# qitianwu/DIFFormer

Hardware: NVIDIA B200
Metric: DIFFormer-layer node-updates/sec (full_attention_conv 'simple', N=132534 H=4 D=64 fp32 per GPU) (higher is better)
Workload: dtype f32

## Files before the change

difformer_b200/csrc/simple_lp_sm100.cu:

```cuda
#include <atomic>
#include <mutex>
#include <vector>

#include "simple_tc.cuh"

namespace dif {
namespace {

constexpr int kLpThreads = 12 * 32;
constexpr int kLpNodes = 32;
constexpr int kLpTile = kLpNodes * 128;
constexpr int kLpNS = 4;
constexpr int kLpQTile = 128 * 128;
constexpr int kLpNQ = 4;
constexpr int kLpOutBox = 32 * 128;
constexpr int kLpOutStage = 4 * 2 * kLpOutBox;

template <int H, bool W = false>
struct LpGeo {
    static constexpr int kStage = 3 * H * kLpTile;
    static constexpr int kSmem1 = kLpNS * kStage;
    static constexpr int kSmem2 = PLay<H, W>::kBBytes + kLpNQ * kLpQTile + kLpOutStage + H * kDim * 4;
    static constexpr int kSmem = (kSmem1 > kSmem2 ? kSmem1 : kSmem2) + 1024;
    static constexpr int kChunks = H * 8;
    static constexpr int kRowGroups = 256 / kChunks;
};

struct Bf16 {
    static constexpr int kFmt = 1;
    __device__ static __forceinline__ void unpack2(uint32_t w, float& a, float& b) { a = __uint_as_float(w << 16); b = __uint_as_float(w & 0xffff0000u); }
    __device__ static __forceinline__ uint32_t pack2(float a, float b) { return bf2_bits(a, b); }
};

__device__ __forceinline__ uint32_t make_idesc_fmt(int M, int N, int a_mn, int b_mn, int a_fmt, int b_fmt) {
    uint32_t d = 0;
    d |= 1u << 4;
    d |= (uint32_t)a_fmt << 7;
    d |= (uint32_t)b_fmt << 10;
    d |= (uint32_t)a_mn << 15;
    d |= (uint32_t)b_mn << 16;
    d |= (uint32_t)(N >> 3) << 17;
    d |= (uint32_t)(M >> 4) << 24;
    return d;
}

struct LpArgs {
    ReduceArgs1 r;
    unsigned long long* flags2;
    int store_hint, reverse, l2_hints, pf_tiles;
};

template <int H, class T, bool W = false>
__global__ void __launch_bounds__(kLpThreads, 1) simple_lp_kernel(const __grid_constant__ LpArgs la, const __grid_constant__ CUtensorMap mq,
                                                                 const __grid_constant__ CUtensorMap mk, const __grid_constant__ CUtensorMap mv,
                                                                 const __grid_constant__ CUtensorMap mo) {
    using G = Geo<H>;
    using L = LpGeo<H, W>;
    using P = PLay<H, W>;
    const ReduceArgs1& a = la.r;
    extern __shared__ uint8_t smem_raw[];
    uint8_t* base = (uint8_t*)(((uintptr_t)smem_raw + 1023) & ~(uintptr_t)1023);
    uint8_t* Bop = base;
    uint8_t* qring = base + P::kBBytes;
    uint8_t* ostage = qring + kLpNQ * kLpQTile;
    float* us = reinterpret_cast<float*>(ostage + kLpOutStage);
    __shared__ uint64_t full[kLpNS], empty[kLpNS], done;
    __shared__ uint64_t qfull[kLpNQ], qempty[kLpNQ], tfull[kNAcc], tempty[kNAcc], bbar;
    __shared__ uint32_t tmem_slot;
    __shared__ float part[16];
    __shared__ __align__(16) float red[H == 1 ? 64 * 65 : 4096];
    const int tid = threadIdx.x, warp = tid >> 5, lane = tid & 31;
    const int64_t r0 = (int64_t)blockIdx.x * a.rows_per_cta;
    const int64_t r1 = min(a.N, r0 + (int64_t)a.rows_per_cta);
    const int iters = r1 > r0 ? (int)((r1 - r0 + kLpNodes - 1) / kLpNodes) : 0;
    const int my_tiles = r1 > r0 ? (int)((r1 - r0 + kTile2 - 1) / kTile2) : 0;
    const int nsc = my_tiles * H;
    auto row0_of = [&](int sc) -> int64_t { const int t = sc / H; return r0 + (int64_t)(la.reverse ? my_tiles - 1 - t : t) * kTile2; };
    uint64_t* dbg = a.dbg;
    DIF_STAMP(dbg, 0);

    if (tid == 0) {
        for (int s = 0; s < kLpNS; ++s) { mbar_init(&full[s], 1); mbar_init(&empty[s], 9); }
// ... 165 lines not shown
                __syncwarp();
                if (lane == 0) mbar_arrive(&empty[s]);
            }
        }
        ssk = warp_sum(ssk);
        ssq = warp_sum(ssq);
        if (lane == 0) { part[warp - 4] = ssk; part[8 + warp - 4] = ssq; }
#pragma unroll
        for (int i = 0; i < 8; ++i) { red[ts * 16 + i] = z[i]; red[ts * 16 + 8 + i] = u[i]; }
        __threadfence_block();
        if (warp >= 8) {
            bar_arrive_named(1, 256);
        } else {
            const int te = tid - 128, ew = warp - 4;
            mbar_wait(&done, 0);
            tc_fence_after();
            bar_sync_named(1, 256);
            if (dbg != nullptr && te == 0) dbg[blockIdx.x * kDbgSlots + 4] = gtime();
            float* rec = a.ws + (int64_t)blockIdx.x * a.ws_len;
            for (int col = te; col < H * kDim; col += 128) {
                const int ccid = col >> 3, e = col & 7;
                float zs = 0.f, usum = 0.f;
                for (int g = 0; g < L::kRowGroups; ++g) { zs += red[(g * L::kChunks + ccid) * 16 + e]; usum += red[(g * L::kChunks + ccid) * 16 + 8 + e]; }
                rec[P::offZ + col] = zs;
                rec[P::offU + col] = usum;
            }
            if (te == 0) {
                float sk = 0.f, sq = 0.f;
                for (int w = 0; w < 8; ++w) { sk += part[w]; sq += part[8 + w]; }
                rec[P::offSq] = sq;
                rec[P::offSq + 1] = sk;
            }
            if (H == 1) bar_sync_named(2, 128);
            const int64_t pf_rows = min((int64_t)min(la.pf_tiles, my_tiles) * kTile2, r1 - r0);
            fused_tail<H, W>(a, la.flags2, rec, te, ew, lane, tmem, iters > 0, red, reinterpret_cast<const __nv_bfloat16*>(a.q) + r0 * (H * kDim),
                          (uint32_t)(max((int64_t)0, pf_rows) * H * kDim * 2));
            if (te == 0) {
                mbar_expect_tx(&bbar, (uint32_t)P::kBBytes);
                for (int i = 0; i < P::kBTiles * 2; ++i)
                    tma_load_1d(smem_u32(Bop) + i * kBOp, a.prepared + (size_t)i * kBOp, (uint32_t)kBOp, &bbar);
            }
            for (int i = te; i < H * kDim; i += 128) us[i] = __ldcg(a.partials + P::offU + i);
            const float cscale = 1.f / (sqrtf(__ldcg(a.partials + P::offSq)) * sqrtf(__ldcg(a.partials + P::offSq + 1)));
            bar_sync_named(2, 128);
            const uint32_t obox = smem_u32(ostage) + ew * 2 * kLpOutBox;
            const uint64_t pol = policy_evict_first();
            float inv_den = 0.f;
            for (int sc = 0; sc < nsc; ++sc) {
                const int64_t trow = row0_of(sc);
                const int h = sc % H, slot = sc % kNAcc;
                mbar_wait(&tfull[slot], (sc / kNAcc) & 1);
                tc_fence_after();
                const uint32_t taddr = tmem + ((uint32_t)(ew * 32) << 16) + slot * kAccCols;
                if (!W || h == 0) {
                    uint32_t qz_bits = tmem_ld1(taddr + kDim);
                    tmem_ld_wait1(qz_bits);
                    inv_den = 1.f / (fmaf(__uint_as_float(qz_bits), cscale, a.n_total));
                }
                const uint32_t ob = obox + (sc & 1) * kLpOutBox;
                if (lane == 0) tma_wait_read1();
                __syncwarp();
#pragma unroll
                for (int c0 = 0; c0 < kDim; c0 += 32) {
                    uint32_t r[32];
                    tmem_ld32(taddr + c0, r);
                    tmem_ld_wait32(r);
                    if (c0 == 32) {
                        tc_fence_before();
                        __syncwarp();
// ... 79 lines not shown
int simple_forward_lp(const void* q, const void* k, const void* v, int dtype, int64_t N, int H, int Hv, int M, int D, double n_total,
                      float* partials, void* out, void* ws, int64_t ws_bytes, cudaStream_t st,
                      void* const* peer_bufs, int rank, int world, unsigned long long seq) {
    const bool wide = simple_wide_supported(N, H, Hv, M, D);
    DIF_REQUIRE(wide || simple_tc_supported(N, H, Hv, M, D), DIF_EUNSUPPORTED, "tcgen05 path: unsupported shape");
    DIF_REQUIRE(dtype == DIF_DTYPE_BF16, DIF_EUNSUPPORTED, "simple_forward(16-bit): bf16 only (dtype %d): up-cast fp16 and use the fp32 kernel", dtype);
    DIF_REQUIRE((((uintptr_t)q | (uintptr_t)k | (uintptr_t)v | (uintptr_t)out) & 15) == 0, DIF_EARG, "simple_forward(16-bit): q/k/v/out must be 16-byte aligned");
    DIF_REQUIRE(((uintptr_t)ws & 127) == 0, DIF_EARG, "simple_forward: workspace must be 128-byte aligned");
    DIF_REQUIRE(N < (1ll << 31), DIF_EUNSUPPORTED, "tcgen05 path: N must fit a 32-bit TMA coordinate");
    int grid;
    const int rpc = tc_rows_per_cta(N, H, &grid);
    const int64_t ws_len = wide ? PLay<2, true>::kWsLen : tc_ws_len(H);
    const int64_t poff = fused_ws_prepared_off(grid, ws_len);
    DIF_REQUIRE(ws_bytes >= poff + (wide ? (int64_t)PLay<2, true>::kBBytes : (int64_t)H * 2 * kBOp), DIF_EARG, "simple_forward: workspace too small");
    DIF_REQUIRE((((ws_len + kSlices - 1) / kSlices + 3) & ~(int64_t)3) <= 128, DIF_EUNSUPPORTED, "simple_forward: slice wider than the tail warps");
    static std::atomic<unsigned long long> epoch_src{0x5851F42D4C957F2Dull ^ (unsigned long long)(uintptr_t)&epoch_src};
    LpArgs la{};
    ReduceArgs1& a = la.r;
    a.N = N; a.rows_per_cta = rpc;
    a.ws = (float*)ws; a.ws_len = ws_len; a.flags = (unsigned long long*)((char*)ws + fused_ws_flags_off(grid, ws_len));
    la.flags2 = a.flags + (int64_t)(grid + 1) * kFlagStride;
    a.epoch = epoch_src.fetch_add(0x632BE59BD9B4E019ull) | 1ull;
    a.partials = partials; a.prepared = (uint8_t*)ws + poff;
    a.n_total = (float)n_total;
    a.sh.world = 1;
    if (peer_bufs != nullptr && world > 1) {
        DIF_REQUIRE(world <= kCommMaxRanks && rank >= 0 && rank < world && seq > 0, DIF_EARG, "simple_forward(sharded): bad rank/world/seq");
        for (int r = 0; r < world; ++r) { DIF_REQUIRE(peer_bufs[r], DIF_EARG, "simple_forward(sharded): null peer buffer"); a.sh.bufs[r] = peer_bufs[r]; }
        a.sh.rank = rank; a.sh.world = world; a.sh.seq = seq;
        a.sh.lenpad = comm_lenpad(SimpleLayout{H, Hv, M, D}.len());
        a.sh.timeout_ns = comm_timeout_ns();
    }
    static const int hints = env_int("DIF_TC_P1_HINTS", 1), sth = env_int("DIF_TC_P2_STORE_HINT", 1), rev = env_int("DIF_TC_FUSED_REVERSE", 1);
    static const int pft = env_int("DIF_TC_FUSED_PF_TILES", 0);
    la.l2_hints = hints; la.store_hint = sth; la.reverse = rev; la.pf_tiles = pft;
    a.q = reinterpret_cast<const float*>(q);
    a.dbg = dbg_buffer();
    const int fp16 = 0;
    CUtensorMap maps[4];
    int rc;
    if ((rc = make_map16(&maps[0], q, N, (int64_t)H * M, fp16))) return rc;
    if ((rc = make_map16(&maps[1], k, N, (int64_t)H * M, fp16))) return rc;
    if ((rc = make_map16(&maps[2], v, N, (int64_t)H * D, fp16))) return rc;
    if ((rc = make_map16(&maps[3], out, N, (int64_t)H * D, fp16))) return rc;
#define DIF_LP(T) (H == 4 ? launch_lp<4, T>(la, maps, grid, st) : H == 2 ? launch_lp<2, T>(la, maps, grid, st) : launch_lp<1, T>(la, maps, grid, st))
    rc = wide ? launch_lp<2, Bf16, true>(la, maps, grid, st) : DIF_LP(Bf16);
#undef DIF_LP
    if (rc) return rc;
    dbg_report("simple_lp", a.dbg, grid);
    return DIF_OK;
}

}
```

difformer_b200/csrc/simple_sm100.cu:

```cuda
#include <stdlib.h>

#include <atomic>
#include <mutex>
#include <vector>

#include "simple_tc.cuh"

namespace dif {

int simple_finalize_fwd(const float* ws, int nchunks, int H, int Hv, int M, int D, float* partials, cudaStream_t st);

namespace {

template <int H, bool BWD>
__global__ void __launch_bounds__(kThreadsT, 1) reduce_tma_kernel(const __grid_constant__ ReduceArgs1 a) {
    using G = Geo<H>;
    extern __shared__ uint8_t smem_raw[];
    uint8_t* stg = (uint8_t*)(((uintptr_t)smem_raw + 1023) & ~(uintptr_t)1023);
    uint8_t* ops = stg + G::kNSG * G::kStg;
    __shared__ uint64_t sfull[G::kNSG], sempty[G::kNSG], ofull[G::kNO], oempty[G::kNO], done, tail_bar;
    __shared__ uint32_t tmem_slot;
    __shared__ float part[16];
    __shared__ __align__(16) float szc[BWD ? H * kDim : 4], su[BWD ? H * kDim : 4];
    const int tid = threadIdx.x, warp = tid >> 5, lane = tid & 31;
// ... 1076 lines not shown
            for (int ks = 0; ks < 4; ++ks) {
                const uint64_t ahi = make_desc(sb + ks * 32, kKmajLBO, kKmajSBO), alo = make_desc(sb + kQOp + ks * 32, kKmajLBO, kKmajSBO);
                const uint64_t bhi = make_desc(bb + ks * 32, kKmajLBO, kKmajSBO), blo = make_desc(bb + kBOpB + ks * 32, kKmajLBO, kKmajSBO);
                umma(d, ahi, bhi, idesc, ks > 0 ? 1u : 0u);
                umma(d, alo, bhi, idesc, 1u);
                umma(d, ahi, blo, idesc, 1u);
            }
            umma_commit(&empty[s]);
            umma_commit(&tfull[slot]);
        }
    }
    __syncwarp();
    tc_fence_before();
    __syncthreads();
    if (warp == 12) tmem_dealloc(tmem, 512);
}


template <int H, bool W = false>
__global__ void __launch_bounds__(kThreadsTC, 1) simple_fused_kernel(const __grid_constant__ FusedArgs fa, const __grid_constant__ CUtensorMap out_map) {
    using G = Geo<H>;
    using P = PLay<H, W>;
    const ReduceArgs1& a = fa.r;
    extern __shared__ uint8_t smem_raw[];
    uint8_t* base = (uint8_t*)(((uintptr_t)smem_raw + 1023) & ~(uintptr_t)1023);
    uint8_t* stg = base;
    uint8_t* ops = stg + G::kNSG * G::kStg;
    uint8_t* Bop = base;
    uint8_t* stages = base + P::kBBytes;
    uint8_t* ostage = stages + kNS2 * kStage2;
    float* us = reinterpret_cast<float*>(ostage + kOutStage);
    __shared__ uint64_t sfull[G::kNSG], sempty[G::kNSG], ofull[G::kNO], oempty[G::kNO], done;
    __shared__ uint64_t full[kNS2], empty[kNS2], tfull[kNAcc], tempty[kNAcc], bbar;
    __shared__ uint32_t tmem_slot;
    __shared__ float part[16];
    __shared__ __align__(16) float red[H == 1 ? 64 * 65 : 2048];
    const int tid = threadIdx.x, warp = tid >> 5, lane = tid & 31;
    const int64_t r0 = (int64_t)blockIdx.x * a.rows_per_cta;
    const int64_t r1 = min(a.N, r0 + (int64_t)a.rows_per_cta);
    const int iters = r1 > r0 ? (int)((r1 - r0 + G::kNodes - 1) / G::kNodes) : 0;
    const int my_tiles = r1 > r0 ? (int)((r1 - r0 + kTile2 - 1) / kTile2) : 0;
    const int nsc = my_tiles * H;
    auto row0_of = [&](int sc) -> int64_t { const int t = sc / H; return r0 + (int64_t)(fa.reverse ? my_tiles - 1 - t : t) * kTile2; };
    uint64_t* dbg = a.dbg;
    DIF_STAMP(dbg, 0);

    if (tid == 0) {
        for (int s = 0; s < G::kNSG; ++s) { mbar_init(&sfull[s], 1); mbar_init(&sempty[s], 8); }
        for (int s = 0; s < G::kNO; ++s) { mbar_init(&ofull[s], 8); mbar_init(&oempty[s], 1); }
        mbar_init(&done, 1);
        for (int s = 0; s < kNS2; ++s) { mbar_init(&full[s], 8); mbar_init(&empty[s], 1); }
        for (int s = 0; s < kNAcc; ++s) { mbar_init(&tfull[s], 1); mbar_init(&tempty[s], 4); }
        mbar_init(&bbar, 1);
        asm volatile("fence.mbarrier_init.release.cluster;" ::: "memory");
    }
    if (warp == 12) tmem_alloc(&tmem_slot, 512);
    tc_fence_before();
    __syncthreads();
    tc_fence_after();
    const uint32_t tmem = tmem_slot;
    pdl_wait();
    DIF_STAMP(dbg, 1);

    if (warp < 8) {
        float zacc[4] = {0.f, 0.f, 0.f, 0.f}, uacc[4] = {0.f, 0.f, 0.f, 0.f};
        float ssk = 0.f, ssq = 0.f;
        {
            const uint32_t stg_base = smem_u32(stg), ops_base = smem_u32(ops);
            for (int it = 0; it < iters; ++it) {
                const int s = it % G::kNSG, o = it % G::kNO;
                const int nrows = (int)min((int64_t)G::kNodes, r1 - (r0 + (int64_t)it * G::kNodes));
                mbar_wait(&sfull[s], (it / G::kNSG) & 1);
                float4 x[G::kChunksPerThread][3];
#pragma unroll
                for (int i = 0; i < G::kChunksPerThread; ++i) {
                    const int u = tid + 256 * i, node = u / G::kChunksPerRow;
#pragma unroll
                    for (int t = 0; t < 3; ++t) {
                        x[i][t] = make_float4(0.f, 0.f, 0.f, 0.f);
                        if (node < nrows) x[i][t] = lds128(stg_base + s * G::kStg + t * G::kStgT + u * 16);
                    }
                }
                if (it >= G::kNO) mbar_wait(&oempty[o], ((it / G::kNO) - 1) & 1);
                const uint32_t ob = ops_base + o * G::kOpStage;
#pragma unroll
                for (int i = 0; i < G::kChunksPerThread; ++i) {
                    const int u = tid + 256 * i, node = u / G::kChunksPerRow, cc = u % G::kChunksPerRow;
                    const int head = cc >> 4, m = (cc & 15) * 4;
                    const int blk = (H == 1) ? (node >> 4) : head;
                    const int kn = (H == 1) ? (node & 15) : node;
                    const uint32_t off = (uint32_t)(blk * G::kBlockTile + (kn >> 3) * 1024 + (kn & 7) * 128 +
                                                    ((((m >> 3) ^ kn) & 7) << 4) + ((m >> 2) & 1) * 8);
                    uint32_t hi[2], lo[2];
                    split4(x[i][0], hi, lo);
                    sts64(ob + 0 * G::kOp + off, hi[0], hi[1]);
                    sts64(ob + 1 * G::kOp + off, lo[0], lo[1]);
                    split4(x[i][1], hi, lo);
                    sts64(ob + 2 * G::kOp + off, hi[0], hi[1]);
                    sts64(ob + 3 * G::kOp + off, lo[0], lo[1]);
                    const float4 kk = x[i][0], vv = x[i][1], qq = x[i][2];
                    zacc[0] += kk.x; zacc[1] += kk.y; zacc[2] += kk.z; zacc[3] += kk.w;
                    uacc[0] += vv.x; uacc[1] += vv.y; uacc[2] += vv.z; uacc[3] += vv.w;
                    ssk = fmaf(kk.x, kk.x, ssk); ssk = fmaf(kk.y, kk.y, ssk); ssk = fmaf(kk.z, kk.z, ssk); ssk = fmaf(kk.w, kk.w, ssk);
                    ssq = fmaf(qq.x, qq.x, ssq); ssq = fmaf(qq.y, qq.y, ssq); ssq = fmaf(qq.z, qq.z, ssq); ssq = fmaf(qq.w, qq.w, ssq);
                }
                fence_proxy_async();
                __syncwarp();
                if (lane == 0) { mbar_arrive(&ofull[o]); mbar_arrive(&sempty[s]); }
            }
        }
        ssk = warp_sum(ssk);
        ssq = warp_sum(ssq);
        if (lane == 0) { part[warp] = ssk; part[8 + warp] = ssq; }
#pragma unroll
        for (int i = 0; i < 4; ++i) { red[tid * 4 + i] = zacc[i]; red[1024 + tid * 4 + i] = uacc[i]; }
        __threadfence_block();
        bar_arrive_named(1, 384);
        float buf[2][4][8];
        auto issue = [&](int sc, int j, float (&dst)[8]) {
            if (sc >= nsc) return;
            const int t = tid + 256 * j;
            const int64_t row = row0_of(sc) + (t >> 3);
            if (row < r1) {
                ldg256_stream(a.q + row * G::kRowF + (sc % H) * kDim + (t & 7) * 8, dst);
            } else {
#pragma unroll
                for (int i = 0; i < 8; ++i) dst[i] = 0.f;
            }
        };
#pragma unroll
        for (int j = 0; j < 4; ++j) issue(0, j, buf[0][j]);
#pragma unroll
        for (int j = 0; j < 4; ++j) issue(1, j, buf[1][j]);
        mbar_wait(&done, 0);
        DIF_STAMP(dbg, 3);
        const uint32_t stage_base = smem_u32(stages);
        for (int sc = 0; sc < nsc; ++sc) {
            const int s = sc % kNS2;
            if (sc >= kNS2) mbar_wait(&empty[s], ((sc / kNS2) - 1) & 1);
            const uint32_t sb = stage_base + s * kStage2;
#pragma unroll
            for (int j = 0; j < 4; ++j) {
                const int t = tid + 256 * j;
                uint4 hi, lo;
                split8(buf[0][j], hi, lo);
                const uint32_t off = sw128(t >> 3, t & 7);
                sts128(sb + off, hi);
                sts128(sb + kQOp + off, lo);
            }
            fence_proxy_async();
            __syncwarp();
            if (lane == 0) mbar_arrive(&full[s]);
#pragma unroll
            for (int j = 0; j < 4; ++j) {
#pragma unroll
                for (int i = 0; i < 8; ++i) buf[0][j][i] = buf[1][j][i];
                issue(sc + 2, j, buf[1][j]);
            }
        }
    } else if (warp < 12) {
        const int te = tid - 256, ew = warp - 8;
        if (warp == 8 && lane == 0) {
            const uint32_t stg_base = smem_u32(stg);
            const uint64_t pol_first = policy_evict_first_(), pol_last = policy_evict_last();
            for (int it = 0; it < iters; ++it) {
                const int s = it % G::kNSG;
                if (it >= G::kNSG) mbar_wait(&sempty[s], ((it / G::kNSG) - 1) & 1);
                const int64_t row = r0 + (int64_t)it * G::kNodes;
                const uint32_t bytes = (uint32_t)(min((int64_t)G::kNodes, r1 - row) * G::kRowB);
                mbar_expect_tx(&sfull[s], 3 * bytes);
                if (a.l2_hints) {
                    tma_load_1d_hint(stg_base + s * G::kStg + 0 * G::kStgT, a.k + row * G::kRowF, bytes, &sfull[s], pol_first);
                    tma_load_1d_hint(stg_base + s * G::kStg + 1 * G::kStgT, a.v + row * G::kRowF, bytes, &sfull[s], pol_first);
                    tma_load_1d_hint(stg_base + s * G::kStg + 2 * G::kStgT, a.q + row * G::kRowF, bytes, &sfull[s], pol_last);
                } else {
                    tma_load_1d(stg_base + s * G::kStg + 0 * G::kStgT, a.k + row * G::kRowF, bytes, &sfull[s]);
                    tma_load_1d(stg_base + s * G::kStg + 1 * G::kStgT, a.v + row * G::kRowF, bytes, &sfull[s]);
                    tma_load_1d(stg_base + s * G::kStg + 2 * G::kStgT, a.q + row * G::kRowF, bytes, &sfull[s]);
                }
            }
        }
        __syncwarp();
        mbar_wait(&done, 0);
        tc_fence_after();
        bar_sync_named(1, 384);
        if (dbg != nullptr && te == 0) dbg[blockIdx.x * kDbgSlots + 4] = gtime();
        float* rec = a.ws + (int64_t)blockIdx.x * a.ws_len;
        for (int col = te; col < G::kRowF; col += 128) {
            float z = 0.f, u = 0.f;
            for (int t = col >> 2; t < 256; t += G::kChunksPerRow) { z += red[t * 4 + (col & 3)]; u += red[1024 + t * 4 + (col & 3)]; }
            rec[P::offZ + col] = z;
            rec[P::offU + col] = u;
        }
        if (te == 0) {
            float sk = 0.f, sq = 0.f;
            for (int w = 0; w < 8; ++w) { sk += part[w]; sq += part[8 + w]; }
            rec[P::offSq] = sq;
            rec[P::offSq + 1] = sk;
        }
        if (H == 1) bar_sync_named(2, 128);
        const int64_t pf_rows = min((int64_t)min(fa.pf_tiles, my_tiles) * kTile2, r1 - r0);
        fused_tail<H, W>(a, fa.flags2, rec, te, ew, lane, tmem, iters > 0, red, a.q + r0 * G::kRowF, (uint32_t)(max((int64_t)0, pf_rows) * G::kRowB));
        if (te == 0) {
            mbar_expect_tx(&bbar, (uint32_t)P::kBBytes);
            for (int i = 0; i < P::kBTiles * 2; ++i)
                tma_load_1d(smem_u32(Bop) + i * kBOp, a.prepared + (size_t)i * kBOp, (uint32_t)kBOp, &bbar);
        }
        for (int i = te; i < H * kDim; i += 128) us[i] = __ldcg(a.partials + P::offU + i);
        const float cscale = 1.f / (sqrtf(__ldcg(a.partials + P::offSq)) * sqrtf(__ldcg(a.partials + P::offSq + 1)));
        bar_sync_named(2, 128);
        const uint32_t obox = smem_u32(ostage) + ew * 2 * kOutBox;
        const uint64_t pol = policy_evict_first();
        float inv_den = 0.f;
        for (int sc = 0; sc < nsc; ++sc) {
            const int64_t trow = row0_of(sc);
            const int h = sc % H, slot = sc % kNAcc;
            mbar_wait(&tfull[slot], (sc / kNAcc) & 1);
            tc_fence_after();
            const uint32_t taddr = tmem + ((uint32_t)(ew * 32) << 16) + slot * kAccCols;
            if (!W || h == 0) {
                uint32_t qz_bits = tmem_ld1(taddr + kDim);
                tmem_ld_wait1(qz_bits);
                inv_den = 1.f / (fmaf(__uint_as_float(qz_bits), cscale, a.n_total));
            }
            if (lane == 0) tma_wait_read0();
            __syncwarp();
#pragma unroll
            for (int c0 = 0; c0 < kDim; c0 += 32) {
                uint32_t r[32];
                tmem_ld32(taddr + c0, r);
                tmem_ld_wait32(r);
                if (c0 == 32) {
                    tc_fence_before();
                    __syncwarp();
                    if (lane == 0) mbar_arrive(&tempty[slot]);
                }
#pragma unroll
                for (int j = 0; j < 32; j += 4) {
                    const float4 u4 = *reinterpret_cast<const float4*>(us + h * kDim + c0 + j);
                    float4 o;
                    o.x = fmaf(__uint_as_float(r[j]), cscale, u4.x) * inv_den;
                    o.y = fmaf(__uint_as_float(r[j + 1]), cscale, u4.y) * inv_den;
                    o.z = fmaf(__uint_as_float(r[j + 2]), cscale, u4.z) * inv_den;
// ... 271 lines not shown
    } else if (shared_a) {
        rc = H == 4 ? launch_apply<4, true>(a, map, grid, st) : launch_apply<2, true>(a, map, grid, st);
    } else {
        rc = H == 4 ? launch_apply<4>(a, map, grid, st) : H == 2 ? launch_apply<2>(a, map, grid, st) : launch_apply<1>(a, map, grid, st);
    }
    if (rc) return rc;
    dbg_report("apply_tc", a.dbg, grid);
    return DIF_OK;
}


bool simple_wide_supported(int64_t N, int H, int Hv, int M, int D) { return N >= 1 && H == 1 && Hv == 1 && M == 128 && D == 128; }

int64_t simple_fused_workspace_bytes(int64_t N, int H, int Hv, int M, int D) {
    const bool wide = simple_wide_supported(N, H, Hv, M, D);
    if (!wide && !simple_tc_supported(N, H, Hv, M, D)) return 0;
    int grid;
    tc_rows_per_cta(N, H, &grid);
    const int64_t ws_len = wide ? PLay<2, true>::kWsLen : tc_ws_len(H);
    return fused_ws_prepared_off(grid, ws_len) + (wide ? (int64_t)PLay<2, true>::kBBytes : (int64_t)H * 2 * kBOp) + 128;
}

template <int H, bool W = false>
static int launch_fused(const FusedArgs& a, const CUtensorMap& map, int grid, cudaStream_t st) {
    static bool attr_set = false;
    if (!attr_set) {
        DIF_CUDA_OK(cudaFuncSetAttribute(simple_fused_kernel<H, W>, cudaFuncAttributeMaxDynamicSharedMemorySize, smem_fused_bytes<H, W>()));
        attr_set = true;
    }
    void* args[] = {(void*)&a, (void*)&map};
    return launch_persistent((const void*)simple_fused_kernel<H, W>, grid, kThreadsTC, (size_t)smem_fused_bytes<H, W>(), st, args);
}

int simple_forward_tc(const float* q, const float* k, const float* v, int64_t N, int H, int Hv, int M, int D, double n_total,
                      float* partials, float* out, void* ws, int64_t ws_bytes, cudaStream_t st,
                      void* const* peer_bufs, int rank, int world, unsigned long long seq) {
    const bool wide = simple_wide_supported(N, H, Hv, M, D);
    DIF_REQUIRE(wide || simple_tc_supported(N, H, Hv, M, D), DIF_EUNSUPPORTED, "tcgen05 path: unsupported shape");
    DIF_REQUIRE((((uintptr_t)q | (uintptr_t)k | (uintptr_t)v) & 31) == 0 && ((uintptr_t)out & 15) == 0, DIF_EARG, "simple_forward: q/k/v must be 32-byte, out 16-byte aligned");
    DIF_REQUIRE(((uintptr_t)ws & 127) == 0, DIF_EARG, "simple_forward: workspace must be 128-byte aligned");
    DIF_REQUIRE(N < (1ll << 31), DIF_EUNSUPPORTED, "tcgen05 path: N must fit a 32-bit TMA coordinate");
    int grid;
    const int rpc = tc_rows_per_cta(N, H, &grid);
    const int64_t ws_len = wide ? PLay<2, true>::kWsLen : tc_ws_len(H);
    const int64_t poff = fused_ws_prepared_off(grid, ws_len);
    DIF_REQUIRE(ws_bytes >= poff + (wide ? (int64_t)PLay<2, true>::kBBytes : (int64_t)H * 2 * kBOp), DIF_EARG, "simple_forward: workspace too small");
    DIF_REQUIRE((((ws_len + kSlices - 1) / kSlices + 3) & ~(int64_t)3) <= 128, DIF_EUNSUPPORTED, "simple_forward: slice wider than the tail warps");
    static std::atomic<unsigned long long> epoch_src{0xA24BAED4963EE407ull ^ (unsigned long long)(uintptr_t)&epoch_src};
    FusedArgs fa{};
    ReduceArgs1& a = fa.r;
    a.q = q; a.k = k; a.v = v; a.N = N; a.rows_per_cta = rpc;
    a.ws = (float*)ws; a.ws_len = ws_len; a.flags = (unsigned long long*)((char*)ws + fused_ws_flags_off(grid, ws_len));
    fa.flags2 = a.flags + (int64_t)(grid + 1) * kFlagStride;
    a.epoch = epoch_src.fetch_add(0x632BE59BD9B4E019ull) | 1ull;
    a.partials = partials; a.prepared = (uint8_t*)ws + poff;
    a.vbar = nullptr;
    static const int hints = env_int("DIF_TC_P1_HINTS", 1), sth = env_int("DIF_TC_P2_STORE_HINT", 1), rev = env_int("DIF_TC_FUSED_REVERSE", 1);
    static const int pft = env_int("DIF_TC_FUSED_PF_TILES", 0);
    a.l2_hints = hints;
    fa.pf_tiles = pft;
    a.n_total = (float)n_total;
    a.sh.world = 1;
    if (peer_bufs != nullptr && world > 1) {
        DIF_REQUIRE(world <= kCommMaxRanks && rank >= 0 && rank < world && seq > 0, DIF_EARG, "simple_forward(sharded): bad rank/world/seq");
        for (int r = 0; r < world; ++r) { DIF_REQUIRE(peer_bufs[r], DIF_EARG, "simple_forward(sharded): null peer buffer"); a.sh.bufs[r] = peer_bufs[r]; }
        a.sh.rank = rank; a.sh.world = world; a.sh.seq = seq;
        a.sh.lenpad = comm_lenpad(SimpleLayout{H, Hv, M, D}.len());
        a.sh.timeout_ns = comm_timeout_ns();
    }
    a.dbg = dbg_buffer();
    fa.out = out; fa.store_hint = sth; fa.reverse = rev;
    CUtensorMap map;
    int rc = make_out_map(&map, out, N, (int64_t)H * D);
    if (rc) return rc;
    rc = wide ? launch_fused<2, true>(fa, map, grid, st)
       : H == 4 ? launch_fused<4>(fa, map, grid, st) : H == 2 ? launch_fused<2>(fa, map, grid, st) : launch_fused<1>(fa, map, grid, st);
    if (rc) return rc;
    dbg_report("simple_fused", a.dbg, grid);
    return DIF_OK;
}

int64_t simple_tc_rowscal_floats(int64_t N, int H) { return N * H * 2; }

int simple_bwd_reduce_tc(const float* q, const float* g, const float* out, const float* partials, double n_total,
                         int64_t N, int H, float* bwd_partials, float* rowscal, void* ws, int64_t ws_bytes, cudaStream_t st) {
    DIF_REQUIRE(simple_tc_supported(N, H, H, kDim, kDim), DIF_EUNSUPPORTED, "tcgen05 path: unsupported shape");
    DIF_REQUIRE((((uintptr_t)q | (uintptr_t)g | (uintptr_t)out) & 15) == 0 && ((uintptr_t)rowscal & 7) == 0, DIF_EARG, "tcgen05 bwd: misaligned pointer");
    int grid;
    const int rpc = tc_rows_per_cta(N, H, &grid);
    const int64_t ws_len = tc_ws_len(H);
    DIF_REQUIRE(ws_bytes >= (int64_t)grid * ws_len * 4 + (int64_t)(grid + 1) * 8, DIF_EARG, "simple_bwd_reduce(tcgen05): workspace too small");
    static std::atomic<unsigned long long> epoch_src{0xD1B54A32D192ED03ull ^ (unsigned long long)(uintptr_t)&epoch_src};
    ReduceArgs1 a{};
// ... 59 lines not shown
```

difformer_b200/csrc/simple_tc.cuh:

```cuda
#pragma once
#include <stdlib.h>

#include "common.cuh"
#include "tc_ptx.cuh"

namespace dif {
namespace {

template <int H>
struct Geo {
    static_assert(H == 1 || H == 2 || H == 4, "tcgen05 path: H in {1, 2, 4}");
    static constexpr int kRowF = H * kDim;
    static constexpr int kRowB = kRowF * 4;
    static constexpr int kBlocks = H < 2 ? 2 : H;
    static constexpr int kPairs = kBlocks / 2;
    static constexpr int kNodes = 16 * kBlocks / H;
    static constexpr int kBlockTile = 16 * 128;
    static constexpr int kOp = kBlocks * kBlockTile;
    static constexpr int kOpStage = 4 * kOp;
    static constexpr int kStgT = kNodes * kRowB;
    static constexpr int kStg = 3 * kStgT;
    static constexpr int kNSG = 3, kNO = 2;
    static constexpr int kSmem1 = kNSG * kStg + kNO * kOpStage + 1024;
    static constexpr int kChunksPerRow = kRowB / 16;
// ... 26 lines not shown
    float* ws;
    int64_t ws_len;
    unsigned long long* flags;
    unsigned long long epoch;
    float* partials;
    uint8_t* prepared;
    int l2_hints;
    ShardArgs sh;
    uint64_t* dbg;
    const float* fwd_partials;
    float n_total;
    float* rowscal;
    float* vbar;
    int gram;
};


constexpr int kTile2 = 128;
constexpr int kQOp = kTile2 * 128;
constexpr int kStage2 = 2 * kQOp;
constexpr int kNS2 = 3;
constexpr int kBN = 80;
constexpr int kNAcc = 4, kAccCols = 128;
constexpr int kOutBox = 32 * 128;
constexpr int kOutStage = 4 * 2 * kOutBox;
template <int H>
constexpr int smem2_bytes() { return Geo<H>::kBBytes + kNS2 * kStage2 + kOutStage + H * kDim * 4 + 1024; }


struct FusedArgs {
    ReduceArgs1 r;
    float* out;
    int store_hint, reverse;
    int pf_tiles;
    unsigned long long* flags2;
};
template <int H, bool W = false>
constexpr int smem_fused_bytes() {
    constexpr int p2 = PLay<H, W>::kBBytes + kNS2 * kStage2 + kOutStage + H * kDim * 4 + 1024;
    return Geo<H>::kSmem1 > p2 ? Geo<H>::kSmem1 : p2;
}

__device__ __forceinline__ void bar_sync_named(int id, int nthreads) { asm volatile("bar.sync %0, %1;" :: "r"(id), "r"(nthreads) : "memory"); }
__device__ __forceinline__ void bar_arrive_named(int id, int nthreads) { asm volatile("bar.arrive %0, %1;" :: "r"(id), "r"(nthreads) : "memory"); }


int tc_grid(int64_t units) {
    const int sms = sm_count();
    return (int)(units < sms ? (units < 1 ? 1 : units) : sms);
}

int tc_rows_per_cta(int64_t N, int H, int* grid) {
    (void)H;
    int g = tc_grid((N + kTile2 - 1) / kTile2);
    int64_t rpc = (N + g - 1) / g;
    rpc = (rpc + kTile2 - 1) / kTile2 * kTile2;
    g = (int)((N + rpc - 1) / rpc);
    *grid = g;
    return (int)rpc;
}

uint64_t* dbg_buffer() {
    static uint64_t* buf = nullptr;
    static int on = -1;
    if (on < 0) { const char* e = getenv("DIF_TC_DEBUG_TIMES"); on = (e && atoi(e)) ? 1 : 0; }
    if (!on) return nullptr;
    if (!buf) cudaMalloc(&buf, 256 * kDbgSlots * sizeof(uint64_t));
    cudaMemset(buf, 0, 256 * kDbgSlots * sizeof(uint64_t));
// ... 49 lines not shown
        return DIF_OK;
    }
    if (mode == 3) {
        cudaLaunchConfig_t cfg{};
        cfg.gridDim = dim3(grid); cfg.blockDim = dim3(threads); cfg.dynamicSmemBytes = smem; cfg.stream = st;
        cudaLaunchAttribute attr[2];
        attr[0].id = cudaLaunchAttributeCooperative;
        attr[0].val.cooperative = 1;
        attr[1].id = cudaLaunchAttributeProgrammaticStreamSerialization;
        attr[1].val.programmaticStreamSerializationAllowed = 1;
        cfg.attrs = attr; cfg.numAttrs = 2;
        DIF_CUDA_OK(cudaLaunchKernelExC(&cfg, kernel, args));
        return DIF_OK;
    }
    int nb = 0;
    DIF_CUDA_OK(cudaOccupancyMaxActiveBlocksPerMultiprocessor(&nb, kernel, threads, smem));
    DIF_REQUIRE(nb >= 1 && grid <= sm_count(), DIF_ECUDA, "persistent kernel cannot be co-resident (grid %d, %d CTA/SM)", grid, nb);
    cudaLaunchConfig_t cfg{};
    cfg.gridDim = dim3(grid); cfg.blockDim = dim3(threads); cfg.dynamicSmemBytes = smem; cfg.stream = st;
    cudaLaunchAttribute attr[1];
    attr[0].id = cudaLaunchAttributeProgrammaticStreamSerialization;
    attr[0].val.programmaticStreamSerializationAllowed = 1;
    cfg.attrs = attr; cfg.numAttrs = mode == 2 ? 1 : 0;
    DIF_CUDA_OK(cudaLaunchKernelExC(&cfg, kernel, args));
    return DIF_OK;
}
__device__ __forceinline__ void pdl_wait() { asm volatile("griddepcontrol.wait;" ::: "memory"); }
__device__ __forceinline__ void pdl_launch_dependents() { asm volatile("griddepcontrol.launch_dependents;" ::: "memory"); }

int64_t tc_ws_len(int H) { return (SimpleLayout{H, H, kDim, kDim}.len() + 7) & ~(int64_t)7; }

constexpr int kFlagStride = 16;
int64_t fused_ws_flags_off(int grid, int64_t ws_len) { return ((int64_t)grid * ws_len * 4 + 127) & ~(int64_t)127; }
int64_t fused_ws_prepared_off(int grid, int64_t ws_len) { return fused_ws_flags_off(grid, ws_len) + (int64_t)(2 * grid + 1) * kFlagStride * 8; }


__device__ __forceinline__ void poll_flags(const unsigned long long* flags, int grid, int l, unsigned long long epoch) {
    constexpr int kMax = 8;
    bool ok;
    do {
        unsigned long long f[kMax];
#pragma unroll
        for (int i = 0; i < kMax; ++i) {
            const int r = l + 32 * i;
            f[i] = epoch;
            if (r < grid) asm volatile("ld.relaxed.gpu.global.u64 %0, [%1];" : "=l"(f[i]) : "l"(flags + (int64_t)r * kFlagStride) : "memory");
        }
        ok = true;
#pragma unroll
        for (int i = 0; i < kMax; ++i) ok = ok && f[i] == epoch;
    } while (!ok);
    __threadfence();
}

template <int H, bool W = false>
__device__ __forceinline__ void fused_tail(const ReduceArgs1& a, unsigned long long* flags2, float* rec, int te, int ew, int lane,
                                           uint32_t tmem, bool have_rows, float* red, const void* pf_ptr = nullptr,
                                           uint32_t pf_bytes = 0) {
    using G = Geo<H>;
    using P = PLay<H, W>;
    uint64_t* dbg = a.dbg;
    if (te == 0)
        for (int64_t i = P::kP; i < a.ws_len; ++i) rec[i] = 0.f;
    if (W) {
        const int m = ew * 32 + lane;
#pragma unroll 1
        for (int cb = 0; cb < 4; ++cb) {
            uint32_t r[32];
            if (have_rows) {
                tmem_ld32(tmem + ((uint32_t)(ew * 32) << 16) + cb * 32, r);
                tmem_ld_wait32(r);
            } else {
#pragma unroll
                for (int j = 0; j < 32; ++j) r[j] = 0u;
            }
            float* dst = rec + (int64_t)m * 128 + cb * 32;
#pragma unroll
            for (int j = 0; j < 32; j += 8)
                asm volatile("st.global.v8.b32 [%0], {%1,%2,%3,%4,%5,%6,%7,%8};"
                             :: "l"(dst + j), "r"(r[j]), "r"(r[j + 1]), "r"(r[j + 2]), "r"(r[j + 3]),
                                "r"(r[j + 4]), "r"(r[j + 5]), "r"(r[j + 6]), "r"(r[j + 7]) : "memory");
        }
    }
#pragma unroll 1
    for (int p = 0; p < (W ? 0 : G::kPairs); ++p) {
        const int wq = ew, hp = wq >> 1, m = (wq * 32 + lane) & 63;
        uint32_t r[2][32];
#pragma unroll
        for (int c = 0; c < 2; ++c) {
            if (have_rows) {
                tmem_ld32(tmem + ((uint32_t)(wq * 32) << 16) + p * 128 + hp * 64 + c * 32, r[c]);
// ... 25 lines not shown
            for (int c = 0; c < 2; ++c)
#pragma unroll
                for (int j = 0; j < 32; j += 8)
                    asm volatile("st.global.v8.b32 [%0], {%1,%2,%3,%4,%5,%6,%7,%8};"
                                 :: "l"(dst + c * 32 + j), "r"(r[c][j]), "r"(r[c][j + 1]), "r"(r[c][j + 2]), "r"(r[c][j + 3]),
                                    "r"(r[c][j + 4]), "r"(r[c][j + 5]), "r"(r[c][j + 6]), "r"(r[c][j + 7]) : "memory");
        }
    }
    tc_fence_before();
    __threadfence();
    bar_sync_named(2, 128);
    if (dbg != nullptr && te == 0) dbg[blockIdx.x * kDbgSlots + 5] = gtime();
    const int grid = gridDim.x;
    const unsigned long long gen = *reinterpret_cast<volatile unsigned long long*>(a.flags + (int64_t)grid * kFlagStride);
    const unsigned long long epoch = a.epoch + gen * 0x9E3779B97F4A7C15ull;
    if (te == 0) asm volatile("st.release.gpu.global.u64 [%0], %1;" :: "l"(a.flags + (int64_t)blockIdx.x * kFlagStride), "l"(epoch) : "memory");
    const int chunk = (int)((((a.ws_len + kSlices - 1) / kSlices) + 3) & ~(int64_t)3);
    const ShardArgs& sh = a.sh;
    const bool sharded = sh.world > 1;
    const int xslot = (int)(sh.seq & 1);
    if (sharded && blockIdx.x == 0 && te == 0) comm_check_status(sh);
    bool waited = false;
    double* gsum = reinterpret_cast<double*>(red);
    for (int sl = blockIdx.x; sl < kSlices; sl += grid) {
        const int64_t j0 = (int64_t)sl * chunk;
        const int slice = (int)max((int64_t)0, min(a.ws_len, j0 + chunk) - j0);
        if (slice <= 0) break;
        if (!waited) {
            if (te < 32) poll_flags(a.flags, grid, te, epoch);
            bar_sync_named(2, 128);
            if (blockIdx.x == 0 && te == 0) *reinterpret_cast<volatile unsigned long long*>(a.flags + (int64_t)grid * kFlagStride) = gen + 1;
            waited = true;
            if (dbg != nullptr && te == 0) dbg[blockIdx.x * kDbgSlots + 8] = gtime();
            if (pf_bytes > 0 && te == 32) {
                for (uint32_t o = 0; o < pf_bytes; o += 32768u)
                    prefetch_l2(reinterpret_cast<const char*>(pf_ptr) + o, min(32768u, pf_bytes - o));
            }
        }
        {
            const int g = te >> 5, l = te & 31;
            double c0 = 0.0, c1 = 0.0, c2 = 0.0, c3 = 0.0;
            if (4 * l < slice) {
                const float* col = a.ws + j0 + 4 * l;
                const int64_t ld = a.ws_len;
                const int gmain = grid & ~3;
                int r = g;
                for (; r + 4 * 18 < gmain; r += 4 * 19) {
                    float4 x[19];
#pragma unroll
                    for (int i = 0; i < 19; ++i) x[i] = __ldcg(reinterpret_cast<const float4*>(col + (int64_t)(r + 4 * i) * ld));
#pragma unroll
                    for (int i = 0; i < 19; ++i) { c0 += (double)x[i].x; c1 += (double)x[i].y; c2 += (double)x[i].z; c3 += (double)x[i].w; }
                }
                for (; r < gmain; r += 4) {
                    const float4 x = __ldcg(reinterpret_cast<const float4*>(col + (int64_t)r * ld));
                    c0 += (double)x.x; c1 += (double)x.y; c2 += (double)x.z; c3 += (double)x.w;
                }
                if (g == 0)
                    for (r = gmain; r < grid; ++r) {
                        const float4 x = __ldcg(reinterpret_cast<const float4*>(col + (int64_t)r * ld));
                        c0 += (double)x.x; c1 += (double)x.y; c2 += (double)x.z; c3 += (double)x.w;
                    }
            }
            if (g > 0) {
                double* d = gsum + (g - 1) * 128 + 4 * l;
                d[0] = c0; d[1] = c1; d[2] = c2; d[3] = c3;
            }
            bar_sync_named(2, 128);
            if (g == 0 && 4 * l < slice) {
                const double* d = gsum + 4 * l;
                float* o = reinterpret_cast<float*>(gsum + 3 * 128);
                o[4 * l + 0] = (float)((c0 + d[0]) + (d[128 + 0] + d[256 + 0]));
                o[4 * l + 1] = (float)((c1 + d[1]) + (d[128 + 1] + d[256 + 1]));
                o[4 * l + 2] = (float)((c2 + d[2]) + (d[128 + 2] + d[256 + 2]));
                o[4 * l + 3] = (float)((c3 + d[3]) + (d[128 + 3] + d[256 + 3]));
            }
            bar_sync_named(2, 128);
        }
        const int64_t j = j0 + te;
        const bool live = te < slice && j < P::kP;
        const float local = live ? reinterpret_cast<const float*>(gsum + 3 * 128)[te] : 0.f;
        float sum = local;
        if (sharded && live) {
            const uint32_t tag = (uint32_t)sh.seq;
            for (int p = 1; p < sh.world; ++p) {
                int r = sh.rank + p;
                if (r >= sh.world) r -= sh.world;
                comm_ll_send(comm_ll_ptr(sh.bufs[r], sh.lenpad, xslot, sh.rank) + j, local, tag);
            }
            sum = comm_ll_sum(sh, xslot, j, tag, local);
        }
        if (live) {
            a.partials[j] = sum;
            if (j < P::offU) {
                int h, n, m;
                if (!W) {
                    if (j < P::offZ) { h = (int)(j >> 12); m = (int)(j >> 6) & 63; n = (int)j & 63; }
                    else { h = (int)(j - P::offZ) >> 6; m = (int)(j - P::offZ) & 63; n = kDim; }
                } else {
                    if (j < P::offZ) { const int mm = (int)(j >> 7), d = (int)j & 127; h = 2 * (d >> 6) + (mm >> 6); m = mm & 63; n = d & 63; }
                    else { const int mm = (int)(j - P::offZ); h = mm >> 6; m = mm & 63; n = kDim; }
                }
                const __nv_bfloat16 hi = __float2bfloat16_rn(sum);
                const __nv_bfloat16 lo = __float2bfloat16_rn(sum - __bfloat162float(hi));
                uint8_t* img = a.prepared + (size_t)h * 2 * kBOp + sw128(n, m >> 3) + (m & 7) * 2;
                *reinterpret_cast<__nv_bfloat16*>(img) = hi;
                *reinterpret_cast<__nv_bfloat16*>(img + kBOp) = lo;
            }
        }
    }
    if (blockIdx.x == grid - 1) {
        for (int i = te; i < P::kBTiles * 2 * 16 * 8; i += 128) {
            const int c = i & 7, rr = (i >> 3) % 16 + 64, t = i / (8 * 16);
            if (rr == 64 && !(W && (t >> 1) >= 2)) continue;
            *reinterpret_cast<uint4*>(a.prepared + (size_t)t * kBOp + sw128(rr, c)) = make_uint4(0u, 0u, 0u, 0u);
        }
    }
    if (dbg != nullptr && te == 0) dbg[blockIdx.x * kDbgSlots + 9] = gtime();
    __threadfence();
    bar_sync_named(2, 128);
    const unsigned long long epoch2 = epoch + 1;
    if (te == 0) asm volatile("st.relaxed.gpu.global.u64 [%0], %1;" :: "l"(flags2 + (int64_t)blockIdx.x * kFlagStride), "l"(epoch2) : "memory");
    if (dbg != nullptr && te == 0) dbg[blockIdx.x * kDbgSlots + 10] = gtime();
    if (te < 32) poll_flags(flags2, grid, te, epoch2);
    asm volatile("fence.proxy.async;" ::: "memory");
    bar_sync_named(2, 128);
    if (dbg != nullptr && te == 0) dbg[blockIdx.x * kDbgSlots + 6] = gtime();
}

}
}
```

Before: 964.6 million.

## Split Q sum-of-squares out of phase A into a late overlapped reduction

When rows per CTA are small, phase A stops loading Q alongside K and V. After publishing the K/V partials, the compute warps stream Q through a separate TMA ring to accumulate the Q sum of squares. That scalar is then reduced across CTAs with its own flag set, so the main grid reduction no longer waits on Q traffic. The unused L2 prefetch-tile option is also removed from both kernels. The cost is an extra grid-wide flag poll and a second pass over Q, which the evict_last hint may keep resident in L2 for phase B.

New measurement: 1.039 billion, median of 6. 1.08x the previous value.

```diff
diff --git a/difformer_b200/csrc/simple_lp_sm100.cu b/difformer_b200/csrc/simple_lp_sm100.cu
--- a/difformer_b200/csrc/simple_lp_sm100.cu
+++ b/difformer_b200/csrc/simple_lp_sm100.cu
@@ -47,7 +47,7 @@
 struct LpArgs {
     ReduceArgs1 r;
     unsigned long long* flags2;
-    int store_hint, reverse, l2_hints, pf_tiles;
+    int store_hint, reverse, l2_hints;
 };
 
 template <int H, class T, bool W = false>
@@ -279,9 +279,7 @@
                 rec[P::offSq + 1] = sk;
             }
             if (H == 1) bar_sync_named(2, 128);
-            const int64_t pf_rows = min((int64_t)min(la.pf_tiles, my_tiles) * kTile2, r1 - r0);
-            fused_tail<H, W>(a, la.flags2, rec, te, ew, lane, tmem, iters > 0, red, reinterpret_cast<const __nv_bfloat16*>(a.q) + r0 * (H * kDim),
-                          (uint32_t)(max((int64_t)0, pf_rows) * H * kDim * 2));
+            fused_tail<H, W>(a, la.flags2, rec, te, ew, lane, tmem, iters > 0, red);
             if (te == 0) {
                 mbar_expect_tx(&bbar, (uint32_t)P::kBBytes);
                 for (int i = 0; i < P::kBTiles * 2; ++i)
@@ -427,9 +425,7 @@
         a.sh.timeout_ns = comm_timeout_ns();
     }
     static const int hints = env_int("DIF_TC_P1_HINTS", 1), sth = env_int("DIF_TC_P2_STORE_HINT", 1), rev = env_int("DIF_TC_FUSED_REVERSE", 1);
-    static const int pft = env_int("DIF_TC_FUSED_PF_TILES", 0);
-    la.l2_hints = hints; la.store_hint = sth; la.reverse = rev; la.pf_tiles = pft;
-    a.q = reinterpret_cast<const float*>(q);
+    la.l2_hints = hints; la.store_hint = sth; la.reverse = rev;
     a.dbg = dbg_buffer();
     const int fp16 = 0;
     CUtensorMap maps[4];
diff --git a/difformer_b200/csrc/simple_sm100.cu b/difformer_b200/csrc/simple_sm100.cu
--- a/difformer_b200/csrc/simple_sm100.cu
+++ b/difformer_b200/csrc/simple_sm100.cu
@@ -1132,6 +1132,10 @@
     float* us = reinterpret_cast<float*>(ostage + kOutStage);
     __shared__ uint64_t sfull[G::kNSG], sempty[G::kNSG], ofull[G::kNO], oempty[G::kNO], done;
     __shared__ uint64_t full[kNS2], empty[kNS2], tfull[kNAcc], tempty[kNAcc], bbar;
+    constexpr int kNQ = (64 << 10) / G::kStgT;
+    static_assert(P::kBBytes + kNQ * G::kStgT <= smem_fused_bytes<H, W>() - 1024, "phase-B ring must fit behind the B image");
+    uint8_t* qring = base + P::kBBytes;
+    __shared__ uint64_t qfull[kNQ], qempty[kNQ];
     __shared__ uint32_t tmem_slot;
     __shared__ float part[16];
     __shared__ __align__(16) float red[H == 1 ? 64 * 65 : 2048];
@@ -1152,6 +1156,7 @@
         for (int s = 0; s < kNS2; ++s) { mbar_init(&full[s], 8); mbar_init(&empty[s], 1); }
         for (int s = 0; s < kNAcc; ++s) { mbar_init(&tfull[s], 1); mbar_init(&tempty[s], 4); }
         mbar_init(&bbar, 1);
+        for (int s = 0; s < kNQ; ++s) { mbar_init(&qfull[s], 1); mbar_init(&qempty[s], 8); }
         asm volatile("fence.mbarrier_init.release.cluster;" ::: "memory");
     }
     if (warp == 12) tmem_alloc(&tmem_slot, 512);
@@ -1161,6 +1166,9 @@
     const uint32_t tmem = tmem_slot;
     pdl_wait();
     DIF_STAMP(dbg, 1);
+    const unsigned long long epoch3 =
+        a.epoch + *reinterpret_cast<volatile unsigned long long*>(a.flags + (int64_t)gridDim.x * kFlagStride) * 0x9E3779B97F4A7C15ull + 2;
+    float* rec = a.ws + (int64_t)blockIdx.x * a.ws_len;
 
     if (warp < 8) {
         float zacc[4] = {0.f, 0.f, 0.f, 0.f}, uacc[4] = {0.f, 0.f, 0.f, 0.f};
@@ -1178,7 +1186,7 @@
 #pragma unroll
                     for (int t = 0; t < 3; ++t) {
                         x[i][t] = make_float4(0.f, 0.f, 0.f, 0.f);
-                        if (node < nrows) x[i][t] = lds128(stg_base + s * G::kStg + t * G::kStgT + u * 16);
+                        if (node < nrows && (t < 2 || !fa.split_q)) x[i][t] = lds128(stg_base + s * G::kStg + t * G::kStgT + u * 16);
                     }
                 }
                 if (it >= G::kNO) mbar_wait(&oempty[o], ((it / G::kNO) - 1) & 1);
@@ -1210,12 +1218,56 @@
             }
         }
         ssk = warp_sum(ssk);
-        ssq = warp_sum(ssq);
-        if (lane == 0) { part[warp] = ssk; part[8 + warp] = ssq; }
+        if (lane == 0) part[warp] = ssk;
 #pragma unroll
         for (int i = 0; i < 4; ++i) { red[tid * 4 + i] = zacc[i]; red[1024 + tid * 4 + i] = uacc[i]; }
         __threadfence_block();
         bar_arrive_named(1, 384);
+        DIF_STAMP(dbg, 11);
+        if (fa.split_q) {
+            const uint32_t qbase = smem_u32(qring);
+            auto issue = [&](int it) {
+                const int s = it % kNQ;
+                const int64_t row = r0 + (int64_t)it * G::kNodes;
+                const uint32_t bytes = (uint32_t)(min((int64_t)G::kNodes, r1 - row) * G::kRowB);
+                mbar_expect_tx(&qfull[s], bytes);
+                tma_load_1d_hint(qbase + s * G::kStgT, a.q + row * G::kRowF, bytes, &qfull[s], policy_evict_last());
+            };
+            if (tid == 0) {
+                mbar_wait(&done, 0);
+                for (int it = 0; it < kNQ && it < iters; ++it) issue(it);
+            }
+            __syncwarp();
+            for (int it = 0; it < iters; ++it) {
+                const int s = it % kNQ;
+                const int nrows = (int)min((int64_t)G::kNodes, r1 - (r0 + (int64_t)it * G::kNodes));
+                mbar_wait(&qfull[s], (it / kNQ) & 1);
+#pragma unroll
+                for (int i = 0; i < G::kChunksPerThread; ++i) {
+                    const int u = tid + 256 * i, node = u / G::kChunksPerRow;
+                    const float4 qq = node < nrows ? lds128(qbase + s * G::kStgT + u * 16) : make_float4(0.f, 0.f, 0.f, 0.f);
+                    ssq = fmaf(qq.x, qq.x, ssq); ssq = fmaf(qq.y, qq.y, ssq); ssq = fmaf(qq.z, qq.z, ssq); ssq = fmaf(qq.w, qq.w, ssq);
+                }
+                __syncwarp();
+                if (lane == 0) mbar_arrive(&qempty[s]);
+                if (tid == 0 && it + kNQ < iters) {
+                    mbar_wait(&qempty[s], (it / kNQ) & 1);
+                    issue(it + kNQ);
+                }
+                __syncwarp();
+            }
+        }
+        ssq = warp_sum(ssq);
+        if (lane == 0) part[8 + warp] = ssq;
+        __threadfence_block();
+        bar_sync_named(3, 256);
+        if (tid == 0) {
+            float sq = 0.f;
+            for (int w = 0; w < 8; ++w) sq += part[8 + w];
+            rec[P::offSq] = sq;
+            asm volatile("st.release.gpu.global.u64 [%0], %1;" :: "l"(fa.flags3 + (int64_t)blockIdx.x * kFlagStride), "l"(epoch3) : "memory");
+        }
+        DIF_STAMP(dbg, 12);
         float buf[2][4][8];
         auto issue = [&](int sc, int j, float (&dst)[8]) {
             if (sc >= nsc) return;
@@ -1263,20 +1315,21 @@
         if (warp == 8 && lane == 0) {
             const uint32_t stg_base = smem_u32(stg);
             const uint64_t pol_first = policy_evict_first_(), pol_last = policy_evict_last();
+            const int nt = fa.split_q ? 2 : 3;
             for (int it = 0; it < iters; ++it) {
                 const int s = it % G::kNSG;
                 if (it >= G::kNSG) mbar_wait(&sempty[s], ((it / G::kNSG) - 1) & 1);
                 const int64_t row = r0 + (int64_t)it * G::kNodes;
                 const uint32_t bytes = (uint32_t)(min((int64_t)G::kNodes, r1 - row) * G::kRowB);
-                mbar_expect_tx(&sfull[s], 3 * bytes);
+                mbar_expect_tx(&sfull[s], nt * bytes);
                 if (a.l2_hints) {
                     tma_load_1d_hint(stg_base + s * G::kStg + 0 * G::kStgT, a.k + row * G::kRowF, bytes, &sfull[s], pol_first);
                     tma_load_1d_hint(stg_base + s * G::kStg + 1 * G::kStgT, a.v + row * G::kRowF, bytes, &sfull[s], pol_first);
-                    tma_load_1d_hint(stg_base + s * G::kStg + 2 * G::kStgT, a.q + row * G::kRowF, bytes, &sfull[s], pol_last);
+                    if (nt == 3) tma_load_1d_hint(stg_base + s * G::kStg + 2 * G::kStgT, a.q + row * G::kRowF, bytes, &sfull[s], pol_last);
                 } else {
                     tma_load_1d(stg_base + s * G::kStg + 0 * G::kStgT, a.k + row * G::kRowF, bytes, &sfull[s]);
                     tma_load_1d(stg_base + s * G::kStg + 1 * G::kStgT, a.v + row * G::kRowF, bytes, &sfull[s]);
-                    tma_load_1d(stg_base + s * G::kStg + 2 * G::kStgT, a.q + row * G::kRowF, bytes, &sfull[s]);
+                    if (nt == 3) tma_load_1d(stg_base + s * G::kStg + 2 * G::kStgT, a.q + row * G::kRowF, bytes, &sfull[s]);
                 }
             }
         }
@@ -1285,7 +1338,6 @@
         tc_fence_after();
         bar_sync_named(1, 384);
         if (dbg != nullptr && te == 0) dbg[blockIdx.x * kDbgSlots + 4] = gtime();
-        float* rec = a.ws + (int64_t)blockIdx.x * a.ws_len;
         for (int col = te; col < G::kRowF; col += 128) {
             float z = 0.f, u = 0.f;
             for (int t = col >> 2; t < 256; t += G::kChunksPerRow) { z += red[t * 4 + (col & 3)]; u += red[1024 + t * 4 + (col & 3)]; }
@@ -1293,22 +1345,22 @@
             rec[P::offU + col] = u;
         }
         if (te == 0) {
-            float sk = 0.f, sq = 0.f;
-            for (int w = 0; w < 8; ++w) { sk += part[w]; sq += part[8 + w]; }
-            rec[P::offSq] = sq;
+            float sk = 0.f;
+            for (int w = 0; w < 8; ++w) sk += part[w];
             rec[P::offSq + 1] = sk;
         }
         if (H == 1) bar_sync_named(2, 128);
-        const int64_t pf_rows = min((int64_t)min(fa.pf_tiles, my_tiles) * kTile2, r1 - r0);
-        fused_tail<H, W>(a, fa.flags2, rec, te, ew, lane, tmem, iters > 0, red, a.q + r0 * G::kRowF, (uint32_t)(max((int64_t)0, pf_rows) * G::kRowB));
+        fused_tail<H, W, true>(a, fa.flags2, rec, te, ew, lane, tmem, iters > 0, red);
         if (te == 0) {
             mbar_expect_tx(&bbar, (uint32_t)P::kBBytes);
             for (int i = 0; i < P::kBTiles * 2; ++i)
                 tma_load_1d(smem_u32(Bop) + i * kBOp, a.prepared + (size_t)i * kBOp, (uint32_t)kBOp, &bbar);
         }
         for (int i = te; i < H * kDim; i += 128) us[i] = __ldcg(a.partials + P::offU + i);
-        const float cscale = 1.f / (sqrtf(__ldcg(a.partials + P::offSq)) * sqrtf(__ldcg(a.partials + P::offSq + 1)));
-        bar_sync_named(2, 128);
+        const float sk = __ldcg(a.partials + P::offSq + 1);
+        const float sq = fused_sq_sum<H, W>(a, fa.flags3, epoch3, te, red);
+        if (dbg != nullptr && te == 0) dbg[blockIdx.x * kDbgSlots + 13] = gtime();
+        const float cscale = 1.f / (sqrtf(sq) * sqrtf(sk));
         const uint32_t obox = smem_u32(ostage) + ew * 2 * kOutBox;
         const uint64_t pol = policy_evict_first();
         float inv_den = 0.f;
@@ -1646,6 +1698,8 @@
     return launch_persistent((const void*)simple_fused_kernel<H, W>, grid, kThreadsTC, (size_t)smem_fused_bytes<H, W>(), st, args);
 }
 
+constexpr int kSplitQRows = 4096;
+
 int simple_forward_tc(const float* q, const float* k, const float* v, int64_t N, int H, int Hv, int M, int D, double n_total,
                       float* partials, float* out, void* ws, int64_t ws_bytes, cudaStream_t st,
                       void* const* peer_bufs, int rank, int world, unsigned long long seq) {
@@ -1666,13 +1720,13 @@
     a.q = q; a.k = k; a.v = v; a.N = N; a.rows_per_cta = rpc;
     a.ws = (float*)ws; a.ws_len = ws_len; a.flags = (unsigned long long*)((char*)ws + fused_ws_flags_off(grid, ws_len));
     fa.flags2 = a.flags + (int64_t)(grid + 1) * kFlagStride;
+    fa.flags3 = fa.flags2 + (int64_t)grid * kFlagStride;
     a.epoch = epoch_src.fetch_add(0x632BE59BD9B4E019ull) | 1ull;
     a.partials = partials; a.prepared = (uint8_t*)ws + poff;
     a.vbar = nullptr;
     static const int hints = env_int("DIF_TC_P1_HINTS", 1), sth = env_int("DIF_TC_P2_STORE_HINT", 1), rev = env_int("DIF_TC_FUSED_REVERSE", 1);
-    static const int pft = env_int("DIF_TC_FUSED_PF_TILES", 0);
     a.l2_hints = hints;
-    fa.pf_tiles = pft;
+    fa.split_q = rpc <= kSplitQRows;
     a.n_total = (float)n_total;
     a.sh.world = 1;
     if (peer_bufs != nullptr && world > 1) {
diff --git a/difformer_b200/csrc/simple_tc.cuh b/difformer_b200/csrc/simple_tc.cuh
--- a/difformer_b200/csrc/simple_tc.cuh
+++ b/difformer_b200/csrc/simple_tc.cuh
@@ -82,8 +82,9 @@
     ReduceArgs1 r;
     float* out;
     int store_hint, reverse;
-    int pf_tiles;
     unsigned long long* flags2;
+    unsigned long long* flags3;
+    int split_q;
 };
 template <int H, bool W = false>
 constexpr int smem_fused_bytes() {
@@ -199,7 +200,7 @@
 
 constexpr int kFlagStride = 16;
 int64_t fused_ws_flags_off(int grid, int64_t ws_len) { return ((int64_t)grid * ws_len * 4 + 127) & ~(int64_t)127; }
-int64_t fused_ws_prepared_off(int grid, int64_t ws_len) { return fused_ws_flags_off(grid, ws_len) + (int64_t)(2 * grid + 1) * kFlagStride * 8; }
+int64_t fused_ws_prepared_off(int grid, int64_t ws_len) { return fused_ws_flags_off(grid, ws_len) + (int64_t)(3 * grid + 1) * kFlagStride * 8; }
 
 
 __device__ __forceinline__ void poll_flags(const unsigned long long* flags, int grid, int l, unsigned long long epoch) {
@@ -220,10 +221,9 @@
     __threadfence();
 }
 
-template <int H, bool W = false>
+template <int H, bool W = false, bool SQ_LATE = false>
 __device__ __forceinline__ void fused_tail(const ReduceArgs1& a, unsigned long long* flags2, float* rec, int te, int ew, int lane,
-                                           uint32_t tmem, bool have_rows, float* red, const void* pf_ptr = nullptr,
-                                           uint32_t pf_bytes = 0) {
+                                           uint32_t tmem, bool have_rows, float* red) {
     using G = Geo<H>;
     using P = PLay<H, W>;
     uint64_t* dbg = a.dbg;
@@ -315,10 +315,6 @@
             if (blockIdx.x == 0 && te == 0) *reinterpret_cast<volatile unsigned long long*>(a.flags + (int64_t)grid * kFlagStride) = gen + 1;
             waited = true;
             if (dbg != nullptr && te == 0) dbg[blockIdx.x * kDbgSlots + 8] = gtime();
-            if (pf_bytes > 0 && te == 32) {
-                for (uint32_t o = 0; o < pf_bytes; o += 32768u)
-                    prefetch_l2(reinterpret_cast<const char*>(pf_ptr) + o, min(32768u, pf_bytes - o));
-            }
         }
         {
             const int g = te >> 5, l = te & 31;
@@ -361,7 +357,7 @@
             bar_sync_named(2, 128);
         }
         const int64_t j = j0 + te;
-        const bool live = te < slice && j < P::kP;
+        const bool live = te < slice && j < P::kP && !(SQ_LATE && j == P::offSq);
         const float local = live ? reinterpret_cast<const float*>(gsum + 3 * 128)[te] : 0.f;
         float sum = local;
         if (sharded && live) {
@@ -411,5 +407,45 @@
     if (dbg != nullptr && te == 0) dbg[blockIdx.x * kDbgSlots + 6] = gtime();
 }
 
-}
-}
+template <int H, bool W = false>
+__device__ __forceinline__ float fused_sq_sum(const ReduceArgs1& a, const unsigned long long* flags3, unsigned long long epoch3, int te,
+                                              float* red) {
+    using P = PLay<H, W>;
+    const int grid = gridDim.x;
+    if (te < 32) {
+        poll_flags(flags3, grid, te, epoch3);
+        for (int r = te; r < grid; r += 32) red[r] = __ldcg(a.ws + (int64_t)r * a.ws_len + P::offSq);
+        __syncwarp();
+        const int gmain = grid & ~3;
+        double c = 0.0;
+        if (te < 4)
+            for (int r = te; r < gmain; r += 4) c += (double)red[r];
+        if (te == 0)
+            for (int r = gmain; r < grid; ++r) c += (double)red[r];
+        const double c1 = __shfl_sync(0xffffffffu, c, 1), c2 = __shfl_sync(0xffffffffu, c, 2), c3 = __shfl_sync(0xffffffffu, c, 3);
+        __syncwarp();
+        if (te == 0) {
+            const float local = (float)((c + c1) + (c2 + c3));
+            float sum = local;
+            const ShardArgs& sh = a.sh;
+            if (sh.world > 1) {
+                const int xslot = (int)(sh.seq & 1);
+                const uint32_t tag = (uint32_t)sh.seq;
+                if (blockIdx.x == 0)
+                    for (int p = 1; p < sh.world; ++p) {
+                        int r = sh.rank + p;
+                        if (r >= sh.world) r -= sh.world;
+                        comm_ll_send(comm_ll_ptr(sh.bufs[r], sh.lenpad, xslot, sh.rank) + P::offSq, local, tag);
+                    }
+                sum = comm_ll_sum(sh, xslot, P::offSq, tag, local);
+            }
+            if (blockIdx.x == 0) a.partials[P::offSq] = sum;
+            red[256] = sum;
+        }
+    }
+    bar_sync_named(2, 128);
+    return red[256];
+}
+
+}
+}
```
